# vpecanins/stm32f7-rtlsdr

Measured on AMD Instinct MI355X. Metric: IQ MSamples/s through FIR+FM-demod+resample, higher is better.
Workload: dtype f32 audio; K2 = u8 x 24-bit fixed-point taps on the i8 matrix pipe, exact i32 sums, one f32 recombination (design Q); K3 / K4 f32; ill-conditioned phases recomputed with the f32 fmaf chain

## Files before the change

include/sdrfm_dev.h:

```cpp
#ifndef SDRFM_DEV_H
#define SDRFM_DEV_H

#include "sdrfm.h"

#ifdef __cplusplus
extern "C" {
#endif

float sdrfm_host_atan2f(float y, float x);
float sdrfm_host_discriminate(float yr, float yi, float pr, float pi);

int sdrfm_debug_discriminate(int device, const float* yr, const float* yi, const float* pr, const float* pi,
                             float* out_scalar, float* out_pair, uint32_t n);

int sdrfm_q_build(const float* h, uint32_t T, uint32_t D, int8_t* A, float* q, float* cst, uint32_t* first_chunk);

int sdrfm_q_guard(const float* h, uint32_t T, const float* g, uint32_t Ta, float* guard_r, float* guard_a);
int sdrfm_q_guard2(const float* h, uint32_t T, const float* g, uint32_t Ta, int worst_case, float* guard_r, float* guard_a);

int sdrfm_debug_q_guard(sdrfm_t* h, float* guard_r, float* guard_a, unsigned long long* lanes, unsigned long long* passes);

int sdrfm_debug_route(sdrfm_t* h, const uint8_t* mask, uint32_t* n_noisy, uint8_t* noisy_out);

int sdrfm_sink_chain_tables(float alpha, float* pc, float* w, float* dinv);

int sdrfm_debug_read_ceiling(int device, const void* const* bufs, uint32_t nbufs, size_t bytes_each, uint32_t passes, double* gbytes_per_s);

int sdrfm_debug_phase_cycles(sdrfm_t* h, unsigned long long* out8);
int sdrfm_debug_raw(sdrfm_t* h, unsigned long long* out560);
int sdrfm_dev_read_debug(sdrfm_t* h, unsigned long long* out, uint32_t n);
// ... 6 lines not shown
```

stm32f7-rtlsdr_amd/csrc/qtaps.c:

```c
#include <math.h>
#include <stdint.h>
#include <string.h>

#include "sdrfm_q_host.h"

int sdrfm_q_build(const float* h, uint32_t T, uint32_t D, int8_t* A, float* q_out, float* cst_out, uint32_t* first_chunk) {
  if (!h || !A || !q_out || !cst_out || !first_chunk) return -1;
  if (D < 2 || (D & 1u) || D > SDRFM_Q_MAX_D || T < 1 || T > 9 * D) return -1;
  double hmax = 0.0, hsum = 0.0;
  for (uint32_t k = 0; k < T; ++k) {
    if (!isfinite(h[k])) return -1;
    if (fabs((double)h[k]) > hmax) hmax = fabs((double)h[k]);
    hsum += (double)h[k];
  }
  if (hmax == 0.0) return -1;
  const double q = hmax / (double)SDRFM_Q_HMAX;
  const float qf = (float)q;
  if (!(qf > 0.0f) || !isfinite(65536.0f * qf)) return -1;
  int8_t dig[SDRFM_Q_DIGITS][9 * SDRFM_Q_MAX_D];
  for (uint32_t k = 0; k < T; ++k) {
    long long H = llround((double)h[k] / (double)qf);
    if (H > SDRFM_Q_HMAX) H = SDRFM_Q_HMAX;
    if (H < -SDRFM_Q_HMAX) H = -SDRFM_Q_HMAX;
    for (int t = 0; t < SDRFM_Q_DIGITS; ++t) {
// ... 13 lines not shown
        const uint32_t h2 = sl >> 3, q4 = (sl >> 1) & 3u, j = sl & 1u;
        const uint32_t kb = 128 * c + 32 * (l >> 4) + 16 * h2 + 4 * q4 + comp + 2 * j;
        const int k = (int)(8 * D + D * o + D - 1) - (int)(kb >> 1);
        if (kb >= 32 * D || k < 0 || k >= (int)T) continue;
        for (int t = 0; t < SDRFM_Q_DIGITS; ++t) {
          A[(((size_t)c * SDRFM_Q_DIGITS + t) * 64 + l) * 16 + sl] = dig[t][k];
          if (dig[t][k] != 0 && c < c0) c0 = c;
        }
      }
  *q_out = qf;
  *cst_out = (float)(0.5 * hsum);
  *first_chunk = c0;
  return 0;
}

int sdrfm_q_guard2(const float* h, uint32_t T, const float* g, uint32_t Ta, int worst_case, float* guard_r, float* guard_a) {
  if (!h || !g || !guard_r || !guard_a || T < 1 || Ta < 1) return -1;
  double habs = 0.0, hmax = 0.0, gmax = 0.0;
  for (uint32_t k = 0; k < T; ++k) { habs += fabs((double)h[k]); if (fabs((double)h[k]) > hmax) hmax = fabs((double)h[k]); }
  for (uint32_t k = 0; k < Ta; ++k) if (fabs((double)g[k]) > gmax) gmax = fabs((double)g[k]);
  if (!isfinite(habs) || !isfinite(gmax)) return -1;
  if (gmax == 0.0) { *guard_r = 0.0f; *guard_a = 4.0f; return 0; }
  const double P = 127.5 * habs, u = ldexp(1.0, -24);
  const double E = worst_case ? ((double)T + 4.0) * P * u + 64.0 * (double)T * (hmax / (double)SDRFM_Q_HMAX)
                              : 1.25 * sqrt((double)T) * P * u;
  *guard_r = (float)(2.0 * gmax * E / 5e-6);
  *guard_a = (float)(3.14159265358979323846 - 2.0 * 5e-6 / gmax);
  return 0;
}

// ... 4 lines not shown
```

stm32f7-rtlsdr_amd/csrc/sdrfm.hip:

```cpp
#include <hip/hip_runtime.h>
#include <hip/hip_ext.h>

#include <cmath>
#include <cstdint>
#include <cstdio>
#include <cstdlib>
#include <cstring>
#include <new>
#include <type_traits>

#include "../../include/sdrfm.h"
#include "../../include/sdrfm_dev.h"
#include "sdrfm_math.h"
#include "sdrfm_q.h"
#include "sdrfm_fm_call.h"
#include "sdrfm_fm_route.h"
#include "sdrfm_fm_plan.h"

#include "sdrfm_b.h"

static_assert(SDRFM_FM_Q_STEP_OUT == SDRFM_Q_STEP_OUT, "sdrfm_fm_call.h counts design Q's steps");
static_assert(SDRFM_FM_CHAIN_FIX == SDRFM_CHAIN_FIX, "sdrfm_fm_call.h sizes the runs of a launch with the sink's chain");

namespace {
// ... 750 lines not shown
  const FastVariant* fast_mix;
  char fast_s_name[64];
  uint32_t AB;
  unsigned long long* d_dbg;
  uint32_t warm_ahead;
  uint32_t dbg_launches;
  int fast_mode;
  uint32_t prio_balance;
  uint32_t end_prio;
  uint32_t stream_profile;
  char kernel_name[112];
  char generic_name[64];
  char fast_name[64];
  int8_t* d_qA;
  float q_scale, q_cst;
  uint32_t q_c0, q_nslot;
  char fast_q_name[64];
  float q_guard_r, q_guard_a;
  float* d_hpad;
  uint8_t* d_hist_q[2];
  unsigned int* d_qstat;
  bool yprev_exact, hist_q_valid;
  bool prev_by_q;
  FmRoute route;
  uint32_t* rt_pass_dev[SDRFM_Q_ADAPT_SETS]; uint32_t* rt_pass_host[SDRFM_Q_ADAPT_SETS]; uint32_t* rt_pass_host_dev[SDRFM_Q_ADAPT_SETS];
  hipStream_t rt_mon;
  hipEvent_t rt_rb_done[SDRFM_Q_ADAPT_SETS];
  hipEvent_t rt_win_evt[SDRFM_Q_ADAPT_SETS][3];
  uint32_t* rt_list_dev[2]; uint32_t* rt_list_host[2];
  hipEvent_t rt_applied[2];
// ... 282 lines not shown
  CR(hipMemcpy(h->d_g, gc, sizeof(float) * Ta, hipMemcpyHostToDevice));
#undef CR

  FmKnobs knobs = fm_read_knobs();
  FmPlanIn in;
  memset(&in, 0, sizeof(in));
  in.T = cfg->fir_taps; in.D = cfg->fir_decim; in.Ta = cfg->audio_taps; in.Da = cfg->audio_decim; in.n_streams = cfg->n_streams;
  in.force_generic = (cfg->flags & SDRFM_CFG_FORCE_GENERIC) != 0; in.bit_exact = (cfg->flags & SDRFM_CFG_BIT_EXACT) != 0;
  in.n_cu = (uint32_t)prop.multiProcessorCount;
  in.q_default_nslot = sdrfm_q_default_nslot(in.D);
  in.q_default_lds = sdrfm_q_lds_bytes(in.q_default_nslot, in.D, in.Da);
  if (!in.force_generic) in.taps = fm_tap_verdict(hc, in.T, gc, in.Ta, (cfg->flags & SDRFM_CFG_GUARD_WORST_CASE) != 0);
  const size_t q_tab_bytes = (size_t)SDRFM_Q_SPARSE_CHUNKS(in.D) * SDRFM_Q_DIGITS * 64 * 16;
  int8_t* q_tab = nullptr;
  float q_scale = 0.f, q_cst = 0.f;
  if (fm_plan_offers_q(in, knobs)) {
    q_tab = (int8_t*)malloc(q_tab_bytes);
    in.q_built = q_tab && sdrfm_q_build(hc, in.T, in.D, q_tab, &q_scale, &q_cst, &in.q_c0) == 0;
    const uint32_t nslot = fm_plan_q_nslot(in, knobs);
    in.q_lds = sdrfm_q_lds_bytes(nslot, in.D, in.Da);
    in.q_symbol = sdrfm_q_kernel_symbol(in.q_c0, nslot, in.D, in.Da);
    in.mix_lds = sdrfm_q_mix_lds(in.q_c0, nslot, in.D, in.Da, in.T, SDRFM_FM_MIX_R);
    if (in.mix_lds) in.mix_blocks_per_cu = sdrfm_q_mix_blocks_per_cu(in.q_c0, nslot, in.D, in.Da, in.T, SDRFM_FM_MIX_R);
  }
  FmRefused refused = {false, 0u};
  FmPlan plan;
  for (;;) {
    plan = fm_plan(in, knobs, refused);
    if (!plan.supported) break;
    if (plan.geo.has_q && !h->d_qA && !q_create(h, q_tab, q_tab_bytes)) {
      fprintf(stderr, "[sdrfm] the matrix-pipe kernel's tables or routing state could not be allocated: this handle runs the bit-exact kernels only\n");
      (void)hipGetLastError();
      q_free(h);
// ... 14 lines not shown
  free(q_tab);
  if (!plan.supported || (plan.lds_bytes > 64 * 1024 && hipFuncSetAttribute(reinterpret_cast<const void*>(k_generic), hipFuncAttributeMaxDynamicSharedMemorySize,
                                                                             (int)plan.lds_bytes) != hipSuccess)) { free_handle(h); return SDRFM_NOT_SUPPORTED; }
  h->geo = plan.geo;
  h->lds_bytes = plan.lds_bytes;
  h->fast = plan.fast >= 0 ? &kFastVariants[plan.fast] : nullptr;
  h->fast_s = plan.fast_s >= 0 ? &kFastVariants[plan.fast_s] : nullptr;
  h->fast_mix = plan.fast_mix >= 0 ? &kFastVariants[plan.fast_mix] : nullptr;
  if (h->geo.has_fast != (h->fast != nullptr) || h->geo.has_s != (h->fast_s != nullptr) || h->geo.has_mix_tile != (h->fast_mix != nullptr)) {
    fprintf(stderr, "[sdrfm] the plan's tiles and its geometry disagree\n");
    free_handle(h);
    return SDRFM_FAIL;
  }
  h->AB = plan.AB; h->warm_ahead = plan.warm_ahead; h->fast_mode = plan.fast_mode; h->stream_profile = plan.stream_profile ? 1u : 0u;
  h->prio_balance = knobs.prio_balance; h->end_prio = knobs.end_prio;
  if (plan.geo.has_q) { h->q_scale = q_scale; h->q_cst = q_cst; }
  h->q_c0 = plan.q_c0; h->q_nslot = plan.q_nslot; h->q_guard_r = plan.q_guard_r; h->q_guard_a = plan.q_guard_a;
  h->rt_off = knobs.q_no_adapt;
  snprintf(h->generic_name, sizeof(h->generic_name), "%s", plan.generic_name);
  snprintf(h->fast_name, sizeof(h->fast_name), "%s", plan.fast_name);
  snprintf(h->fast_s_name, sizeof(h->fast_s_name), "%s", plan.fast_s_name);
  snprintf(h->fast_q_name, sizeof(h->fast_q_name), "%s", plan.fast_q_name);
  snprintf(h->kernel_name, sizeof(h->kernel_name), "%s", plan.kernel_name);
  const int rc = sdrfm_reset(h);
  if (rc != SDRFM_OK) { free_handle(h); return rc; }
  *out = h;
  return SDRFM_OK;
}

void sdrfm_destroy(sdrfm_t* h) {
  if (!h) return;
// ... 303 lines not shown
  if (q_ok) {
    const uint32_t q_steps = fm_q_steps(M);
    SdrfmQParams q;
    q.iq_prev = nullptr; q.iq_prev_stride = 0; q.N_prev = 0;
    if (ovl) { q.iq_prev = h->prev_iq; q.iq_prev_stride = h->prev_stride; q.N_prev = h->prev_nbytes / 2; }
    q.iq = d_iq; q.iq_stride = iq_stride; q.audio = d_audio; q.audio_stride = audio_stride;
    q.yprev_in = p.yprev_in; q.yprev_out = p.yprev_out; q.hist_d_in = p.hist_d_in; q.hist_d_out = p.hist_d_out;
    q.hist_b_in = p.hist_b_in; q.hist_b_out = p.hist_b_out; q.hist_x_out = p.hist_x_out;
    q.A = h->d_qA; q.g = h->d_g; q.q0 = h->q_scale; q.q2 = 65536.0f * h->q_scale; q.cst = h->q_cst;
    q.T = c.fir_taps; q.N = N; q.M = M; q.A_out = A; q.steps_total = q_steps; q.n_streams = n_clean; q.dbg = nullptr; q.prio_by_age = ovl ? 0u : 1u;
    q.slist = list_dev;
    if (!h->hist_q_valid && !ovl && c.fir_taps > 1)
      HIP_TRY(hipMemcpy2DAsync(h->d_hist_q[h->cur] + 2 * (SDRFM_Q_TP - (c.fir_taps - 1)), 2 * SDRFM_Q_TP, p.hist_b_in, 2 * (size_t)(c.fir_taps - 1),
                               2 * (size_t)(c.fir_taps - 1), c.n_streams, hipMemcpyDeviceToDevice, h->stream), SDRFM_FAIL);
    q.hpad = h->d_hpad; q.hist_q_in = h->d_hist_q[h->cur]; q.hist_q_out = h->d_hist_q[h->cur ^ 1];
    q.guard_r = h->q_guard_r; q.guard_a = h->q_guard_a; q.yprev_exact = h->yprev_exact ? 1u : 0u; q.n_repaired = h->d_qstat;
    const FmRuns r = fm_q_runs(cl, split.q_total, n_clean, with_chain, h->runstate_cap, fm_chain_run_quads(g.Da));
    q.runs = r.runs;
    const bool carry = ovl && h->ovl_join_style;
    const FmRouteStop stop = fm_route_stop(rt, counting, k, carry);
    q.stream_pass = counting ? h->rt_pass_dev[stop.set] : nullptr;
    const hipEvent_t done = stop.evt == FM_ROUTE_OVL_DONE ? h->ovl_done[k] : stop.evt == FM_ROUTE_WINDOW_EVENT ? h->rt_win_evt[stop.set][k] : nullptr;
    with_chain = r.with_chain;
    if (with_chain) {
      chain.pcm = h->pcm_out; chain.pcm_stride = h->pcm_out_stride;
      if (h->pcm_no_audio) q.audio = nullptr;
      chain.run_call = h->chain_calls++;
      chain.runstate = h->d_runstate + (size_t)(chain.run_call % SDRFM_CHAIN_SETS) * h->runstate_cap;
    }
    if (fuse && with_chain) {
      HIP_TRY(sdrfm_q_launch_mix_pcm(q, chain, h->q_c0, h->q_nslot, c.fir_decim, c.audio_decim, pb, pb_blocks, g.mix_R, qs, nullptr), SDRFM_FAIL);
// ... 377 lines not shown
```

stm32f7-rtlsdr_amd/csrc/sdrfm_q.h:

```cpp
#ifndef SDRFM_Q_H
#define SDRFM_Q_H

#include <hip/hip_runtime.h>
#include <stdint.h>

#include "sdrfm_q_host.h"
#include "sdrfm_sink_chain.h"

struct SdrfmQParams {
  const uint8_t* iq;
  size_t iq_stride;
  const uint8_t* iq_prev;
  size_t iq_prev_stride;
  uint32_t N_prev;
  float* audio;
  size_t audio_stride;
  const float2* yprev_in;
  float2* yprev_out;
  const float* hist_d_in;
  float* hist_d_out;
  const uint8_t* hist_b_in;
  uint8_t* hist_b_out;
  float2* hist_x_out;
  const int8_t* A;
  const float* g;
  float q0, q2, cst;
  uint32_t T;
  uint32_t N, M, A_out;
  uint32_t steps_total;
  uint32_t runs;
  uint32_t n_streams;
  uint32_t prio_by_age;
  const float* hpad;
  const uint8_t* hist_q_in;
  uint8_t* hist_q_out;
  float guard_r;
  float guard_a;
  uint32_t yprev_exact;
  unsigned int* n_repaired;
  unsigned int* stream_pass;
  const uint32_t* slist;
  unsigned long long* dbg;
};

#define SDRFM_Q_D 10u
#define SDRFM_Q_DA 5u
#define SDRFM_Q_STEP_OUT 128u

bool sdrfm_q_geometry_ok(uint32_t d, uint32_t da);
uint32_t sdrfm_q_default_nslot(uint32_t d);
uint32_t sdrfm_q_lds_bytes(uint32_t nslot, uint32_t d, uint32_t da);
int sdrfm_q_blocks_per_cu(uint32_t first_chunk, uint32_t nslot, uint32_t d, uint32_t da);
hipError_t sdrfm_q_launch(const SdrfmQParams& p, uint32_t first_chunk, uint32_t nslot, uint32_t d, uint32_t da, hipStream_t stream, hipEvent_t done = nullptr);
bool sdrfm_q_has_pcm_chain(uint32_t first_chunk, uint32_t nslot, uint32_t d, uint32_t da);
hipError_t sdrfm_q_launch_pcm(const SdrfmQParams& p, const SdrfmSinkChain& t, uint32_t first_chunk, uint32_t nslot, uint32_t d, uint32_t da, hipStream_t stream,
                              hipEvent_t done = nullptr);
const char* sdrfm_q_kernel_symbol(uint32_t first_chunk, uint32_t nslot, uint32_t d, uint32_t da);
struct CallParams;
uint32_t sdrfm_q_mix_lds(uint32_t first_chunk, uint32_t nslot, uint32_t d, uint32_t da, uint32_t T, uint32_t b_R);
int sdrfm_q_mix_blocks_per_cu(uint32_t first_chunk, uint32_t nslot, uint32_t d, uint32_t da, uint32_t T, uint32_t b_R);
hipError_t sdrfm_q_launch_mix(const SdrfmQParams& q, uint32_t first_chunk, uint32_t nslot, uint32_t d, uint32_t da, const CallParams& b, uint32_t b_blocks,
                              uint32_t b_R, hipStream_t stream, hipEvent_t done);
hipError_t sdrfm_q_launch_mix_pcm(const SdrfmQParams& q, const SdrfmSinkChain& t, uint32_t first_chunk, uint32_t nslot, uint32_t d, uint32_t da, const CallParams& b,
                                  uint32_t b_blocks, uint32_t b_R, hipStream_t stream, hipEvent_t done);
hipError_t sdrfm_q_fix_yprev(const uint8_t* hist_q, const float* hpad, float2* yprev, uint32_t n_streams, const uint32_t* list, hipStream_t stream);

#endif
```

stm32f7-rtlsdr_amd/csrc/sdrfm_q.hip:

```cpp
#include <hip/hip_runtime.h>
#include <hip/hip_ext.h>

#include <cstddef>
#include <cstdint>
#include <type_traits>

#include "sdrfm_math.h"
#include "sdrfm_q.h"
#include "sdrfm_b.h"

typedef int qi4_t __attribute__((ext_vector_type(4)));
typedef int qi8_t __attribute__((ext_vector_type(8)));
typedef float qf2_t __attribute__((ext_vector_type(2)));
__device__ void q_raw_buffer_load_lds(qi4_t rsrc, __attribute__((address_space(3))) void* lds, int size, int voffset, int soffset,
                                      int offset, int aux) __asm("llvm.amdgcn.raw.buffer.load.lds");

namespace {

constexpr int QTA = (int)SDRFM_Q_TA;
constexpr int DB0 = 128;
constexpr int ABS = 4;
constexpr int ABW = 128 * ABS;
constexpr int FLW = 64 + 2;
#ifndef SDRFM_Q_GTAB
// ... 20 lines not shown
#ifndef SDRFM_Q_HO_RING
#define SDRFM_Q_HO_RING 1
#endif
#ifndef SDRFM_Q_K3
#define SDRFM_Q_K3 1
#endif
#ifndef SDRFM_Q_XORSKIP
#define SDRFM_Q_XORSKIP 1
#endif
#ifndef SDRFM_Q_PEEL
#define SDRFM_Q_PEEL 1
#endif
#ifndef SDRFM_Q_MICRO
#define SDRFM_Q_MICRO 1
#endif
#ifndef SDRFM_Q_AUX
#define SDRFM_Q_AUX 2
#endif
#ifndef SDRFM_Q_WQB
#define SDRFM_Q_WQB 4
#endif
constexpr int WQB = SDRFM_Q_WQB;
static_assert(WQB >= 4 && WQB <= 16 && 8 * WQB >= (int)SDRFM_Q_TA, "a warm-up holds the d history of a run's first audio output");

__device__ __forceinline__ float q_discriminate(float yr, float yi, float pr, float pi) {
  const float re = __builtin_fmaf(yr, pr, yi * pi);
  const float im = yi * pr - yr * pi;
  const float ax = __builtin_fabsf(re), ay = __builtin_fabsf(im);
  const float mx = __builtin_fmaxf(__builtin_fmaxf(ax, ay), 0x1p-120f), mn = __builtin_fminf(ax, ay);
  const float v = mn * __builtin_amdgcn_rcpf(mx);
  const float s2 = v * v;
  float q = 0x1.e34882p-8f;
  q = __builtin_fmaf(q, s2, -0x1.22fc74p-5f);
  q = __builtin_fmaf(q, s2, 0x1.509024p-4f);
  q = __builtin_fmaf(q, s2, -0x1.12688cp-3f);
  q = __builtin_fmaf(q, s2, 0x1.96c562p-3f);
  q = __builtin_fmaf(q, s2, -0x1.554086p-2f);
  float a = __builtin_fmaf(v, s2 * q, v);
  if (ay > ax) a = 0x1.921fb6p+0f - a;
  if (re < 0.0f) a = 0x1.921fb6p+1f - a;
  return __builtin_copysignf(a, im);
}

__device__ __forceinline__ float q_angle(float yr, float yi, float& mx_out) {
  const float ax = __builtin_fabsf(yr), ay = __builtin_fabsf(yi);
  const float mx = __builtin_fmaxf(__builtin_fmaxf(ax, ay), 0x1p-120f), mn = __builtin_fminf(ax, ay);
  mx_out = mx;
  const float v = mn * __builtin_amdgcn_rcpf(mx);
  const float s2 = v * v;
  float q = 0x1.e34882p-8f;
  q = __builtin_fmaf(q, s2, -0x1.22fc74p-5f);
  q = __builtin_fmaf(q, s2, 0x1.509024p-4f);
  q = __builtin_fmaf(q, s2, -0x1.12688cp-3f);
  q = __builtin_fmaf(q, s2, 0x1.96c562p-3f);
  q = __builtin_fmaf(q, s2, -0x1.554086p-2f);
  float a = __builtin_fmaf(v, s2 * q, v);
  if (ay > ax) a = 0x1.921fb6p+0f - a;
  if (yr < 0.0f) a = 0x1.921fb6p+1f - a;
  return __builtin_copysignf(a, yi);
}
__device__ __forceinline__ float q_wrap(float x) {
  float t = __builtin_fmaf(x, 0x1.45f306p-3f, 0x1.8p+23f);
  asm volatile("" : "+v"(t));
  const float k = t - 0x1.8p+23f;
  return __builtin_fmaf(k, -0x1.921fb6p+2f, x);
}

__device__ __forceinline__ unsigned q_pcm_word(float v) {
  const float c = __builtin_amdgcn_fmed3f(v, -32768.0f, 32767.0f);
  float t = c + 0x1.8p+23f;
  asm volatile("" : "+v"(t));
  return __builtin_amdgcn_perm(__builtin_bit_cast(unsigned, t), __builtin_bit_cast(unsigned, t), 0x05040504u);
}

template <int N>
__device__ __forceinline__ void wait_vmcnt() {
  static_assert(N >= 0 && N < 16, "vmcnt immediate");
  __builtin_amdgcn_s_waitcnt(0x0f70 | N);
}

// ... 144 lines not shown
    constexpr int HSW = ALIGNED ? 0x70 : 0;
#ifdef SDRFM_Q_LDSXOR
    hb0 ^= 0x8080; hb1 ^= 0x8080;
#endif
    if (lane < HT) *reinterpret_cast<unsigned short*>(smem + ((PRE - 2 * HT + 2 * lane) ^ HSW)) = hb0;
    if (lane + 64 < HT) *reinterpret_cast<unsigned short*>(smem + ((PRE - 2 * HT + 2 * (lane + 64)) ^ HSW)) = hb1;
    if (lane < QTA - 1) db[DB0 + sigma - (QTA - 1) + lane] = hd0;
  }
#if SDRFM_Q_K3
  float cth = 0.0f;
  unsigned long long cfl = 0ull;
  if (!warm) {
    float mxp;
    const float tp = q_angle(cr, ci, mxp);
    cth = __builtin_bit_cast(float, __builtin_amdgcn_readfirstlane(__builtin_bit_cast(int, tp)));
    cfl = __builtin_amdgcn_ballot_w64(mxp < p.guard_r) & 1ull;
  }
#endif
  db[lane] = hz0;
  if (lane < 2 * QD) db[64 + lane] = hz1;
#if SDRFM_Q_GTAB
  if (lane < QTA) gt[lane] = gt0;
#endif
  __builtin_amdgcn_wave_barrier();
  int slot = 0;
  int ringoff = 0;
  int osm = 0;
  int mbase = o0;
  const int baddr = BLKB * n + 16 * g;
  int rdoff[ALIGNED ? 2 * NSC : 1];
  if constexpr (ALIGNED) {
// ... 31 lines not shown
    t_wait += __builtin_readcyclecounter() - tw0;
    if (t_first == 0) t_first = __builtin_amdgcn_s_memrealtime();
#endif
    if constexpr (ALIGNED) {
      const int ro0 = n == 0 ? 0 : ringoff;
#pragma unroll
      for (int c = 2 * C0; c < 2 * NSC; ++c) dst[c - 2 * C0] = *reinterpret_cast<const qi4_t*>(smem + rdoff[c] + (64 * c < BLKB ? ro0 : ringoff));
      if (lane < BLKB / 16) {
        const qi4_t hcp = *reinterpret_cast<const qi4_t*>(smem + PRE + ringoff + STEPB - BLKB + 16 * lane);
        *reinterpret_cast<qi4_t*>(smem + 16 * lane) = hcp;
      }
      __builtin_amdgcn_wave_barrier();
    } else {
      const unsigned char* wb = smem + baddr + ringoff;
#pragma unroll
      for (int c = 2 * C0; c < 2 * NSC; ++c) dst[c - 2 * C0] = *reinterpret_cast<const qi4_t*>(wb + 64 * c);
      if (ringoff + STEPB == RINGB) {
        if (lane < BLKB / 16) {
          const qi4_t hcp = *reinterpret_cast<const qi4_t*>(smem + PRE + RINGB - BLKB + 16 * lane);
          *reinterpret_cast<qi4_t*>(smem + 16 * lane) = hcp;
        }
        __builtin_amdgcn_wave_barrier();
      }
    }
    if constexpr (RINGB == 2 * STEPB) ringoff ^= STEPB;
    else ringoff = (ringoff + STEPB == RINGB) ? 0 : ringoff + STEPB;
  };
  auto refill_step = [&](int k) {
    asm volatile("s_waitcnt lgkmcnt(0)" ::: "memory");
    if constexpr (ALIGNED) {
#pragma unroll
// ... 216 lines not shown
        float* dst = db + DB0 + sigma + 128 * slot + 8 * (l & 15) + 2 * (l >> 4);
        dst[0] = sdrfm_discriminate(a[1].x, a[1].y, a[0].x, a[0].y);
        dst[1] = sdrfm_discriminate(a[2].x, a[2].y, a[1].x, a[1].y);
      }
    }
    R_PHASE(7, 0, 1);
    if (ln == 0) {
      cnt[0] += nrep;
      cnt[1] += 1u;
    }
    nflag = 0;
    R_PHASE(7, 32, 1);
  };
#ifdef SDRFM_Q_GUARD_L1
  float guard_r = 2.0f * p.guard_r, guard_a = p.guard_a;
#else
  float guard_r = p.guard_r, guard_a = p.guard_a;
#endif
  asm volatile("" : "+v"(guard_r), "+v"(guard_a));
#ifdef SDRFM_Q_SCALE_VGPR
  float q0v = p.q0, q2v = p.q2, cstv = p.cst;
  asm volatile("" : "+v"(q0v), "+v"(q2v), "+v"(cstv));
#else
  const float q0v = p.q0, q2v = p.q2, cstv = p.cst;
#endif
#if SDRFM_Q_MICRO && SDRFM_Q_K3
  int doff = (PRE + RINGB) + 4 * (DB0 + sigma + dlane);
  asm volatile("" : "+v"(doff));
#endif
  const int wrank = (int)(__builtin_amdgcn_s_getreg((3 << 11) | 4) & 15u);
  const int prio_at = p.prio_by_age ? nsteps / 2 : -1;
#if SDRFM_Q_PEEL
  auto step = [&](auto LAST_, const int kk) {
    constexpr bool LAST = decltype(LAST_)::value;
#else
  for (int kk = 0; kk < nsteps; ++kk) {
    const bool LAST = kk == nsteps - 1;
#endif
    if (kk == prio_at) {
// ... 18 lines not shown
        if (lane < 2 * QTP / 16)
          *reinterpret_cast<qi4_t*>(pp->hist_q_out + (size_t)(2 * QTP) * stream + 16 * lane) =
              *reinterpret_cast<const qi4_t*>(smem + PRE + ((Ge - 2 * QTP + 16 * lane) % RINGB));
      }
    }
#endif
    Q_PHASE(1);
    if (!(SDRFM_Q_PEEL && LAST)) refill_step(kk);
#ifdef SDRFM_Q_EARLYSTORE
    if (LAST && npend > 0) flush_audio();
#endif
    Q_PHASE(2);
    qi4_t acc[SDRFM_Q_DIGITS];
#pragma unroll
    for (int t = 0; t < SDRFM_Q_DIGITS; ++t) acc[t] = qi4_t{0, 0, 0, 0};
    [[maybe_unused]] constexpr int XM = (int)0x80808080;
#ifndef SDRFM_Q_LDSXOR
#pragma unroll
    for (int c = 0; c < NB - 1 + (NCH & 1 ? 0 : 1); ++c)
      B[c] = B[c] ^ ((SDRFM_Q_XORSKIP && QD == 10 && C0 == 0 && c == 0) ? qi4_t{0, XM, XM, XM} : qi4_t{XM, XM, XM, XM});
#endif
#pragma unroll
    for (int c = C0; c < NSC; ++c) {
      const qi4_t lo = B[2 * c - 2 * C0], hi = B[2 * c + 1 - 2 * C0];
      const qi8_t b = {lo.x, lo.y, lo.z, lo.w, hi.x, hi.y, hi.z, hi.w};
#pragma unroll
      for (int t = 0; t < SDRFM_Q_DIGITS; ++t) {
#if defined(SDRFM_Q_ABLATE) && (SDRFM_Q_ABLATE & 2)
        acc[t] += At[c - C0][t] & lo;
#else
        acc[t] = __builtin_amdgcn_smfmac_i32_16x16x128_i8(At[c - C0][t], b, acc[t], sidx, 0, 0);
#endif
      }
    }
    float y[4];
#pragma unroll
    for (int r = 0; r < 4; ++r) {
      const int s01 = acc[0][r] + acc[1][r] * 256;
      y[r] = __builtin_fmaf((float)s01, q0v, __builtin_fmaf((float)acc[2][r], q2v, cstv));
    }
#ifdef SDRFM_Q_PHASES
    asm volatile("" : "+v"(y[0]), "+v"(y[1]), "+v"(y[2]), "+v"(y[3]));
#endif
    Q_PHASE(3);
#if SDRFM_Q_K3
    float mx0, mx1;
    const float th1 = q_angle(y[2], y[3], mx1);
    float thp = __builtin_bit_cast(float, __builtin_amdgcn_ds_bpermute(srcaddr, __builtin_bit_cast(int, th1)));
    const float th0 = q_angle(y[0], y[1], mx0);
#if SDRFM_Q_MICRO
    asm("v_writelane_b32 %0, %1, 0" : "+v"(thp) : "s"(cth));
#else
    if (lane == 0) thp = cth;
#endif
#ifdef SDRFM_Q_PHASES
    asm volatile("" : "+v"(thp));
#endif
    Q_PHASE(4);
    cth = __builtin_bit_cast(float, __builtin_amdgcn_readlane(__builtin_bit_cast(int, th1), 63));
    const float d1 = q_wrap(th1 - th0);
    const float d0 = q_wrap(th0 - thp);
#else
    float pr = __builtin_bit_cast(float, __builtin_amdgcn_ds_bpermute(srcaddr, __builtin_bit_cast(int, y[2])));
    float pi = __builtin_bit_cast(float, __builtin_amdgcn_ds_bpermute(srcaddr, __builtin_bit_cast(int, y[3])));
    if (lane == 0) { pr = cr; pi = ci; }
#ifdef SDRFM_Q_PHASES
    asm volatile("" : "+v"(pr), "+v"(pi));
#endif
    Q_PHASE(4);
    cr = __builtin_bit_cast(float, __builtin_amdgcn_readlane(__builtin_bit_cast(int, y[2]), 63));
    ci = __builtin_bit_cast(float, __builtin_amdgcn_readlane(__builtin_bit_cast(int, y[3]), 63));
#if defined(SDRFM_Q_ABLATE) && (SDRFM_Q_ABLATE & 1)
    const float d0 = y[0] + pr + y[1] * pi, d1 = y[2] + y[3] * y[1] + y[0];
#else
    const float d1 = q_discriminate(y[2], y[3], y[0], y[1]);
    const float d0 = q_discriminate(y[0], y[1], pr, pi);
// ... 197 lines not shown
  }
#ifdef SDRFM_Q_STAMPS
  if (tsp && lane == 0) {
    tsp[0] = t_entry; tsp[1] = t_first; tsp[2] = t_loop; tsp[3] = __builtin_amdgcn_s_memrealtime(); tsp[4] = t_wait;
#ifdef SDRFM_Q_PHASES
    for (int i = 0; i < 8; ++i) tsp[8 + i] = t_ph[i];
#endif
    tsp[5] = (__builtin_amdgcn_s_getreg((3 << 11) | 20) & 7) | ((unsigned long long)__builtin_amdgcn_s_getreg((31 << 11) | 4) << 8);
    tsp[6] = (unsigned long long)nsteps; tsp[7] = __builtin_readcyclecounter() - c_entry;
  }
#endif
}


template <int C0, int NSLOT, int D, int DA>
__global__ void __launch_bounds__(64) __attribute__((amdgpu_waves_per_eu(D == 16 ? 3 : 4))) k_mfir(SdrfmQParams p) {
  mfir_body<C0, NSLOT, D, DA>(p, blockIdx.x);
}

template <int C0, int NSLOT, int D, int DA>
__global__ void __launch_bounds__(64) __attribute__((amdgpu_waves_per_eu(D == 16 ? 3 : 4))) k_mfir_pcm(QPcmArgs a) {
  mfir_body<C0, NSLOT, D, DA, true>(a.p, blockIdx.x);
}

template <int C0, int NSLOT, int D, int DA, int T, int R>
__global__ void __launch_bounds__(64) __attribute__((amdgpu_waves_per_eu(3, 4))) k_mix(SdrfmQParams q, CallParams b, uint32_t nb) {
  if (blockIdx.x < nb) fastb_body<T, D, R, (int)SDRFM_Q_TA, DA, 0>(b, blockIdx.x);
  else mfir_body<C0, NSLOT, D, DA>(q, blockIdx.x - nb);
}

struct MixPcmArgs { QPcmArgs qa; CallParams b; uint32_t nb; };
template <int C0, int NSLOT, int D, int DA, int T, int R>
__global__ void __launch_bounds__(64) __attribute__((amdgpu_waves_per_eu(3, 4))) k_mix_pcm(MixPcmArgs a) {
  if (blockIdx.x < a.nb) fastb_body<T, D, R, (int)SDRFM_Q_TA, DA, 0>(a.b, blockIdx.x);
  else mfir_body<C0, NSLOT, D, DA, true>(a.qa.p, blockIdx.x - a.nb);
}
// ... 107 lines not shown
}

uint32_t sdrfm_q_default_nslot(uint32_t d) { return d == 10 ? 5u : (d == 8 ? 4u : (d == 16 ? 8u : 0u)); }

bool sdrfm_q_geometry_ok(uint32_t d, uint32_t da) { return q_find(0, sdrfm_q_default_nslot(d), d, da) != nullptr; }

uint32_t sdrfm_q_lds_bytes(uint32_t nslot, uint32_t d, uint32_t da) {
  const QVariant* v = q_find(0, nslot, d, da);
  return v ? v->lds : 0u;
}

const char* sdrfm_q_kernel_symbol(uint32_t first_chunk, uint32_t nslot, uint32_t d, uint32_t da) {
  const QVariant* v = q_find(first_chunk, nslot, d, da);
  return v ? v->name : "";
}

int sdrfm_q_blocks_per_cu(uint32_t first_chunk, uint32_t nslot, uint32_t d, uint32_t da) {
  const QVariant* v = q_find(first_chunk, nslot, d, da);
  int nb = 0;
  if (!v || hipOccupancyMaxActiveBlocksPerMultiprocessor(&nb, reinterpret_cast<const void*>(v->k), 64, v->lds) != hipSuccess) return 0;
  return nb;
}

hipError_t sdrfm_q_fix_yprev(const uint8_t* hist_q, const float* hpad, float2* yprev, uint32_t n_streams, const uint32_t* list, hipStream_t stream) {
  hipLaunchKernelGGL(k_q_fix_yprev, dim3((n_streams + 63) / 64), dim3(64), 0, stream, hist_q, hpad, yprev, n_streams, list);
  return hipGetLastError();
}

hipError_t sdrfm_q_launch(const SdrfmQParams& p, uint32_t first_chunk, uint32_t nslot, uint32_t d, uint32_t da, hipStream_t stream, hipEvent_t done) {
  const QVariant* v = q_find(first_chunk, nslot, d, da);
// ... 57 lines not shown
```

stm32f7-rtlsdr_amd/csrc/sdrfm_q_host.h:

```cpp
#ifndef SDRFM_Q_HOST_H
#define SDRFM_Q_HOST_H

#include <stdint.h>

#ifdef __cplusplus
extern "C" {
#endif

#define SDRFM_Q_DIGITS 3
#define SDRFM_Q_HMAX (127 * 65793)
#define SDRFM_Q_MAX_D 16

#define SDRFM_Q_TA 32u
#define SDRFM_Q_TP 64u
#define SDRFM_Q_SPARSE_CHUNKS(D) (((D) + 3u) / 4u)

int sdrfm_q_build(const float* h, uint32_t T, uint32_t D, int8_t* A, float* q, float* cst, uint32_t* first_chunk);

int sdrfm_q_guard(const float* h, uint32_t T, const float* g, uint32_t Ta, float* guard_r, float* guard_a);
int sdrfm_q_guard2(const float* h, uint32_t T, const float* g, uint32_t Ta, int worst_case, float* guard_r, float* guard_a);

#ifdef __cplusplus
}
#endif
#endif
```

stm32f7-rtlsdr_amd/lib.py:

```python
import ctypes as C
import os

import numpy as np

_HERE = os.path.dirname(os.path.abspath(__file__))

STATUS = {
    0: "SDRFM_OK", 1: "SDRFM_BUSY", 2: "SDRFM_FAIL", 3: "SDRFM_NOT_SUPPORTED", 4: "SDRFM_UNRECOVERED_ERROR",
    16: "SDRFM_EINVAL", 17: "SDRFM_EODD", 18: "SDRFM_ECAPACITY", 19: "SDRFM_NO_DEVICE", 20: "SDRFM_ENOMEM",
}
OK, EINVAL, EODD, ECAPACITY, NO_DEVICE = 0, 16, 17, 18, 19
F_DEVICE_PTRS = 1
F_OVERLAP = 2
TUNE_SHARED_INPUT = 1

ABI_SYMBOLS = [
    "sdrfm_create", "sdrfm_destroy", "sdrfm_reset", "sdrfm_audio_count", "sdrfm_process", "sdrfm_process_batch",
    "sdrfm_set_stream", "sdrfm_synchronize", "sdrfm_flush", "sdrfm_flush_previous", "sdrfm_wait_previous", "sdrfm_process_batch_pcm", "sdrfm_kernel_name", "sdrfm_abi_version", "sdrfm_strerror",
    "sdrfm_wbfm_create", "sdrfm_wbfm_destroy", "sdrfm_wbfm_reset", "sdrfm_wbfm_audio_count", "sdrfm_wbfm_process_batch",
    "sdrfm_wbfm_set_stream", "sdrfm_wbfm_synchronize", "sdrfm_wbfm_kernel_name", "sdrfm_rtl_pack_fir", "sdrfm_rtl_resampler", "sdrfm_e4k_pll_params",
    "sdrfm_shard_range",
    "sdrfm_spectrum_create", "sdrfm_spectrum_destroy", "sdrfm_spectrum_process_batch", "sdrfm_spectrum_set_stream",
    "sdrfm_spectrum_synchronize", "sdrfm_spectrum_kernel_name",
    "sdrfm_pcm_deemph_s16", "sdrfm_pcm_alpha",
# ... 18 lines not shown
    "sdrfm_bcast_process_batch_metered_hist", "sdrfm_bcast_hist_kernel_name",
    "sdrfm_pcm_audio_meter_s16", "sdrfm_audio_meter_add", "sdrfm_audio_meter_report",
    "sdrfm_pcm_stereo_sink_meter_enable", "sdrfm_pcm_stereo_sink_meter_disable", "sdrfm_pcm_stereo_sink_meter_read",
    "sdrfm_loudness_default_coef", "sdrfm_loudness_check_coef", "sdrfm_loudness_check_domain", "sdrfm_pcm_loudness_s16", "sdrfm_loudness_gate_create", "sdrfm_loudness_gate_push",
    "sdrfm_loudness_gate_report", "sdrfm_loudness_gate_reset", "sdrfm_loudness_gate_free", "sdrfm_pcm_stereo_sink_loudness_enable",
    "sdrfm_pcm_stereo_sink_loudness_disable", "sdrfm_pcm_stereo_sink_loudness_read", "sdrfm_pcm_stereo_sink_loudness_get_state",
    "sdrfm_truepeak_default_coef", "sdrfm_truepeak_check_coef", "sdrfm_truepeak_limit", "sdrfm_pcm_truepeak_s16", "sdrfm_truepeak_add",
    "sdrfm_truepeak_report", "sdrfm_pcm_stereo_sink_truepeak_enable", "sdrfm_pcm_stereo_sink_truepeak_disable",
    "sdrfm_pcm_stereo_sink_truepeak_read",
    "sdrfm_pcm_rate_create", "sdrfm_pcm_rate_destroy", "sdrfm_pcm_rate_reset", "sdrfm_pcm_rate_set_step", "sdrfm_pcm_rate_count",
    "sdrfm_pcm_rate_process_batch", "sdrfm_pcm_rate_get_state", "sdrfm_pcm_rate_set_stream", "sdrfm_pcm_rate_synchronize",
    "sdrfm_pcm_rate_kernel_name", "sdrfm_pcm_rate_s16", "sdrfm_pcm_rate_check_coef",
]


TEST_HOOK_SYMBOLS = ["sdrfm_host_atan2f", "sdrfm_host_discriminate", "sdrfm_debug_discriminate", "sdrfm_q_build", "sdrfm_q_guard", "sdrfm_q_guard2", "sdrfm_debug_q_guard", "sdrfm_debug_read_ceiling", "sdrfm_debug_route", "sdrfm_sink_chain_tables"]
DEV_ONLY_SYMBOLS = ["sdrfm_debug_phase_cycles", "sdrfm_debug_raw", "sdrfm_dev_read_debug"]


class SdrfmError(RuntimeError):
    def __init__(self, status, where=""):
        self.status = int(status)
        name = STATUS.get(self.status, "status %d" % self.status)
        msg = ""
        try:
            msg = load_library().sdrfm_strerror(self.status).decode()
        except Exception:
            pass
        super().__init__("%s%s (%s)" % (where + ": " if where else "", name, msg))


# ... 196 lines not shown
    lib.sdrfm_strerror.argtypes = [C.c_int]
    lib.sdrfm_strerror.restype = C.c_char_p
    lib.sdrfm_host_atan2f.argtypes = [C.c_float, C.c_float]
    lib.sdrfm_host_atan2f.restype = C.c_float
    lib.sdrfm_host_discriminate.argtypes = [C.c_float] * 4
    lib.sdrfm_host_discriminate.restype = C.c_float
    lib.sdrfm_sink_chain_tables.argtypes = [C.c_float] + [C.POINTER(C.c_float)] * 3
    lib.sdrfm_sink_chain_tables.restype = C.c_int
    if dev:
        lib.sdrfm_debug_phase_cycles.argtypes = [vp, C.POINTER(C.c_uint64)]
        lib.sdrfm_debug_phase_cycles.restype = C.c_int
        lib.sdrfm_debug_raw.argtypes = [vp, C.POINTER(C.c_uint64)]
        lib.sdrfm_debug_raw.restype = C.c_int
    lib.sdrfm_q_build.argtypes = [vp, u32, u32, vp, C.POINTER(C.c_float), C.POINTER(C.c_float), u32p]
    lib.sdrfm_q_build.restype = C.c_int
    lib.sdrfm_debug_discriminate.argtypes = [C.c_int] + [vp] * 6 + [u32]
    lib.sdrfm_debug_discriminate.restype = C.c_int
    lib.sdrfm_q_guard.argtypes = [vp, u32, vp, u32, C.POINTER(C.c_float), C.POINTER(C.c_float)]
    lib.sdrfm_q_guard.restype = C.c_int
    lib.sdrfm_q_guard2.argtypes = [vp, u32, vp, u32, C.c_int, C.POINTER(C.c_float), C.POINTER(C.c_float)]
    lib.sdrfm_q_guard2.restype = C.c_int
    lib.sdrfm_debug_read_ceiling.argtypes = [C.c_int, C.POINTER(vp), u32, C.c_size_t, u32, C.POINTER(C.c_double)]
    lib.sdrfm_debug_read_ceiling.restype = C.c_int
    lib.sdrfm_debug_q_guard.argtypes = [vp, C.POINTER(C.c_float), C.POINTER(C.c_float), C.POINTER(C.c_uint64), C.POINTER(C.c_uint64)]
    lib.sdrfm_debug_q_guard.restype = C.c_int
    lib.sdrfm_debug_route.argtypes = [vp, C.POINTER(C.c_uint8), C.POINTER(C.c_uint32), C.POINTER(C.c_uint8)]
    lib.sdrfm_debug_route.restype = C.c_int
    lib.sdrfm_wbfm_create.argtypes = [C.POINTER(WbfmConfig), C.POINTER(vp)]
    lib.sdrfm_wbfm_create.restype = C.c_int
    lib.sdrfm_wbfm_destroy.argtypes = [vp]
# ... 274 lines not shown
```

Measured before the change: 2.558 million.

## Recombine Q-path FIR sums scale-free with integer seed and drop dead B-chunk load

Drops the per-output float scale and constant from the design-Q recombination. The 0.5*sum(h) constant becomes an integer seed, computed on the host and preloaded into the digit-0 accumulator. Because K3 works on differences of angles, the output is only combined as acc0 + 256*acc1 + 65536*acc2, and the guard radius is rescaled by the quantum to match. It also skips loading the last, all-zero B half-chunk when the chunk count is odd, and adds optional knobs for pinning constants to VGPRs and for occupancy, both off by default. The aim is fewer VALU ops and fewer LDS reads per step, at the cost of an int32 overflow check and a changed scale for the yprev history.

```diff
diff --git a/include/sdrfm_dev.h b/include/sdrfm_dev.h
--- a/include/sdrfm_dev.h
+++ b/include/sdrfm_dev.h
@@ -14,6 +14,8 @@
                              float* out_scalar, float* out_pair, uint32_t n);
 
 int sdrfm_q_build(const float* h, uint32_t T, uint32_t D, int8_t* A, float* q, float* cst, uint32_t* first_chunk);
+
+int sdrfm_q_seed(const float* h, uint32_t T, uint32_t D, int32_t* seed);
 
 int sdrfm_q_guard(const float* h, uint32_t T, const float* g, uint32_t Ta, float* guard_r, float* guard_a);
 int sdrfm_q_guard2(const float* h, uint32_t T, const float* g, uint32_t Ta, int worst_case, float* guard_r, float* guard_a);
diff --git a/stm32f7-rtlsdr_amd/csrc/qtaps.c b/stm32f7-rtlsdr_amd/csrc/qtaps.c
--- a/stm32f7-rtlsdr_amd/csrc/qtaps.c
+++ b/stm32f7-rtlsdr_amd/csrc/qtaps.c
@@ -1,5 +1,6 @@
 #include <math.h>
 #include <stdint.h>
+#include <stdlib.h>
 #include <string.h>
 
 #include "sdrfm_q_host.h"
@@ -51,6 +52,37 @@
   return 0;
 }
 
+int sdrfm_q_seed(const float* h, uint32_t T, uint32_t D, int32_t* seed_out) {
+  if (!h || !seed_out || D < 2 || (D & 1u) || D > SDRFM_Q_MAX_D || T < 1 || T > 9 * D) return -1;
+  double hmax = 0.0, hsum = 0.0;
+  for (uint32_t k = 0; k < T; ++k) {
+    if (!isfinite(h[k])) return -1;
+    if (fabs((double)h[k]) > hmax) hmax = fabs((double)h[k]);
+    hsum += (double)h[k];
+  }
+  if (hmax == 0.0) return -1;
+  const float qf = (float)(hmax / (double)SDRFM_Q_HMAX);
+  if (!(qf > 0.0f) || !isfinite(65536.0f * qf)) return -1;
+  long long sumH = 0, reach = 0;
+  for (uint32_t k = 0; k < T; ++k) {
+    long long H = llround((double)h[k] / (double)qf);
+    if (H > SDRFM_Q_HMAX) H = SDRFM_Q_HMAX;
+    if (H < -SDRFM_Q_HMAX) H = -SDRFM_Q_HMAX;
+    sumH += H;
+    const long long d0 = ((H + 128) % 256 + 256) % 256 - 128, H1 = (H - d0) / 256, d1 = ((H1 + 128) % 256 + 256) % 256 - 128;
+    reach += 128 * (llabs(d0) + 256 * llabs(d1));
+  }
+  long long seed = sumH / 2;
+  if (sumH & 1) {
+    const double want = 0.5 * hsum / (double)qf;
+    const long long lo = (sumH - 1) / 2;
+    seed = fabs((double)lo - want) <= fabs((double)(lo + 1) - want) ? lo : lo + 1;
+  }
+  if (llabs(seed) + reach > 2147483647LL) return -1;
+  *seed_out = (int32_t)seed;
+  return 0;
+}
+
 int sdrfm_q_guard2(const float* h, uint32_t T, const float* g, uint32_t Ta, int worst_case, float* guard_r, float* guard_a) {
   if (!h || !g || !guard_r || !guard_a || T < 1 || Ta < 1) return -1;
   double habs = 0.0, hmax = 0.0, gmax = 0.0;
diff --git a/stm32f7-rtlsdr_amd/csrc/sdrfm.hip b/stm32f7-rtlsdr_amd/csrc/sdrfm.hip
--- a/stm32f7-rtlsdr_amd/csrc/sdrfm.hip
+++ b/stm32f7-rtlsdr_amd/csrc/sdrfm.hip
@@ -788,6 +788,7 @@
   char fast_name[64];
   int8_t* d_qA;
   float q_scale, q_cst;
+  int32_t q_seed;
   uint32_t q_c0, q_nslot;
   char fast_q_name[64];
   float q_guard_r, q_guard_a;
@@ -1100,9 +1101,10 @@
   const size_t q_tab_bytes = (size_t)SDRFM_Q_SPARSE_CHUNKS(in.D) * SDRFM_Q_DIGITS * 64 * 16;
   int8_t* q_tab = nullptr;
   float q_scale = 0.f, q_cst = 0.f;
+  int32_t q_seed = 0;
   if (fm_plan_offers_q(in, knobs)) {
     q_tab = (int8_t*)malloc(q_tab_bytes);
-    in.q_built = q_tab && sdrfm_q_build(hc, in.T, in.D, q_tab, &q_scale, &q_cst, &in.q_c0) == 0;
+    in.q_built = q_tab && sdrfm_q_build(hc, in.T, in.D, q_tab, &q_scale, &q_cst, &in.q_c0) == 0 && sdrfm_q_seed(hc, in.T, in.D, &q_seed) == 0;
     const uint32_t nslot = fm_plan_q_nslot(in, knobs);
     in.q_lds = sdrfm_q_lds_bytes(nslot, in.D, in.Da);
     in.q_symbol = sdrfm_q_kernel_symbol(in.q_c0, nslot, in.D, in.Da);
@@ -1147,7 +1149,7 @@
   }
   h->AB = plan.AB; h->warm_ahead = plan.warm_ahead; h->fast_mode = plan.fast_mode; h->stream_profile = plan.stream_profile ? 1u : 0u;
   h->prio_balance = knobs.prio_balance; h->end_prio = knobs.end_prio;
-  if (plan.geo.has_q) { h->q_scale = q_scale; h->q_cst = q_cst; }
+  if (plan.geo.has_q) { h->q_scale = q_scale; h->q_cst = q_cst; h->q_seed = q_seed; }
   h->q_c0 = plan.q_c0; h->q_nslot = plan.q_nslot; h->q_guard_r = plan.q_guard_r; h->q_guard_a = plan.q_guard_a;
   h->rt_off = knobs.q_no_adapt;
   snprintf(h->generic_name, sizeof(h->generic_name), "%s", plan.generic_name);
@@ -1481,7 +1483,7 @@
       HIP_TRY(hipMemcpy2DAsync(h->d_hist_q[h->cur] + 2 * (SDRFM_Q_TP - (c.fir_taps - 1)), 2 * SDRFM_Q_TP, p.hist_b_in, 2 * (size_t)(c.fir_taps - 1),
                                2 * (size_t)(c.fir_taps - 1), c.n_streams, hipMemcpyDeviceToDevice, h->stream), SDRFM_FAIL);
     q.hpad = h->d_hpad; q.hist_q_in = h->d_hist_q[h->cur]; q.hist_q_out = h->d_hist_q[h->cur ^ 1];
-    q.guard_r = h->q_guard_r; q.guard_a = h->q_guard_a; q.yprev_exact = h->yprev_exact ? 1u : 0u; q.n_repaired = h->d_qstat;
+    q.guard_r = h->q_guard_r; q.guard_a = h->q_guard_a; q.seed = h->q_seed; q.guard_rq = h->q_guard_r / h->q_scale; q.yprev_exact = h->yprev_exact ? 1u : 0u; q.n_repaired = h->d_qstat;
     const FmRuns r = fm_q_runs(cl, split.q_total, n_clean, with_chain, h->runstate_cap, fm_chain_run_quads(g.Da));
     q.runs = r.runs;
     const bool carry = ovl && h->ovl_join_style;
diff --git a/stm32f7-rtlsdr_amd/csrc/sdrfm_q.h b/stm32f7-rtlsdr_amd/csrc/sdrfm_q.h
--- a/stm32f7-rtlsdr_amd/csrc/sdrfm_q.h
+++ b/stm32f7-rtlsdr_amd/csrc/sdrfm_q.h
@@ -36,6 +36,8 @@
   uint8_t* hist_q_out;
   float guard_r;
   float guard_a;
+  int32_t seed;
+  float guard_rq;
   uint32_t yprev_exact;
   unsigned int* n_repaired;
   unsigned int* stream_pass;
@@ -56,6 +58,7 @@
 hipError_t sdrfm_q_launch_pcm(const SdrfmQParams& p, const SdrfmSinkChain& t, uint32_t first_chunk, uint32_t nslot, uint32_t d, uint32_t da, hipStream_t stream,
                               hipEvent_t done = nullptr);
 const char* sdrfm_q_kernel_symbol(uint32_t first_chunk, uint32_t nslot, uint32_t d, uint32_t da);
+double sdrfm_q_yprev_scale(float q0);
 struct CallParams;
 uint32_t sdrfm_q_mix_lds(uint32_t first_chunk, uint32_t nslot, uint32_t d, uint32_t da, uint32_t T, uint32_t b_R);
 int sdrfm_q_mix_blocks_per_cu(uint32_t first_chunk, uint32_t nslot, uint32_t d, uint32_t da, uint32_t T, uint32_t b_R);
diff --git a/stm32f7-rtlsdr_amd/csrc/sdrfm_q.hip b/stm32f7-rtlsdr_amd/csrc/sdrfm_q.hip
--- a/stm32f7-rtlsdr_amd/csrc/sdrfm_q.hip
+++ b/stm32f7-rtlsdr_amd/csrc/sdrfm_q.hip
@@ -58,6 +58,19 @@
 #ifndef SDRFM_Q_MICRO
 #define SDRFM_Q_MICRO 1
 #endif
+#ifndef SDRFM_Q_SCALEFREE
+#define SDRFM_Q_SCALEFREE 1
+#endif
+#ifndef SDRFM_Q_NOB6
+#define SDRFM_Q_NOB6 1
+#endif
+#ifndef SDRFM_Q_CVGPR
+#define SDRFM_Q_CVGPR 0
+#endif
+#ifndef SDRFM_Q_W3
+#define SDRFM_Q_W3 0
+#endif
+static_assert(!SDRFM_Q_SCALEFREE || SDRFM_Q_K3, "the scale-free recombination rests on K3 as a difference of angles");
 #ifndef SDRFM_Q_AUX
 #define SDRFM_Q_AUX 2
 #endif
@@ -86,28 +99,35 @@
   return __builtin_copysignf(a, im);
 }
 
-__device__ __forceinline__ float q_angle(float yr, float yi, float& mx_out) {
+struct QK {
+  float c[6] = {0x1.e34882p-8f, -0x1.22fc74p-5f, 0x1.509024p-4f, -0x1.12688cp-3f, 0x1.96c562p-3f, -0x1.554086p-2f};
+  float w[3] = {0x1.45f306p-3f, 0x1.8p+23f, -0x1.921fb6p+2f};
+  float hpi = 0x1.921fb6p+0f, pi = 0x1.921fb6p+1f;
+  float k16 = 65536.0f;
+  int xm = (int)0x80808080;
+};
+__device__ __forceinline__ float q_angle(float yr, float yi, float& mx_out, const QK& K = QK{}) {
   const float ax = __builtin_fabsf(yr), ay = __builtin_fabsf(yi);
   const float mx = __builtin_fmaxf(__builtin_fmaxf(ax, ay), 0x1p-120f), mn = __builtin_fminf(ax, ay);
   mx_out = mx;
   const float v = mn * __builtin_amdgcn_rcpf(mx);
   const float s2 = v * v;
-  float q = 0x1.e34882p-8f;
-  q = __builtin_fmaf(q, s2, -0x1.22fc74p-5f);
-  q = __builtin_fmaf(q, s2, 0x1.509024p-4f);
-  q = __builtin_fmaf(q, s2, -0x1.12688cp-3f);
-  q = __builtin_fmaf(q, s2, 0x1.96c562p-3f);
-  q = __builtin_fmaf(q, s2, -0x1.554086p-2f);
+  float q = K.c[0];
+  q = __builtin_fmaf(q, s2, K.c[1]);
+  q = __builtin_fmaf(q, s2, K.c[2]);
+  q = __builtin_fmaf(q, s2, K.c[3]);
+  q = __builtin_fmaf(q, s2, K.c[4]);
+  q = __builtin_fmaf(q, s2, K.c[5]);
   float a = __builtin_fmaf(v, s2 * q, v);
-  if (ay > ax) a = 0x1.921fb6p+0f - a;
-  if (yr < 0.0f) a = 0x1.921fb6p+1f - a;
+  if (ay > ax) a = K.hpi - a;
+  if (yr < 0.0f) a = K.pi - a;
   return __builtin_copysignf(a, yi);
 }
-__device__ __forceinline__ float q_wrap(float x) {
-  float t = __builtin_fmaf(x, 0x1.45f306p-3f, 0x1.8p+23f);
+__device__ __forceinline__ float q_wrap(float x, const QK& K = QK{}) {
+  float t = __builtin_fmaf(x, K.w[0], K.w[1]);
   asm volatile("" : "+v"(t));
-  const float k = t - 0x1.8p+23f;
-  return __builtin_fmaf(k, -0x1.921fb6p+2f, x);
+  const float k = t - K.w[1];
+  return __builtin_fmaf(k, K.w[2], x);
 }
 
 __device__ __forceinline__ unsigned q_pcm_word(float v) {
@@ -282,7 +302,11 @@
     float mxp;
     const float tp = q_angle(cr, ci, mxp);
     cth = __builtin_bit_cast(float, __builtin_amdgcn_readfirstlane(__builtin_bit_cast(int, tp)));
+#if SDRFM_Q_SCALEFREE
+    cfl = __builtin_amdgcn_ballot_w64(mxp < (p.yprev_exact ? p.guard_r : p.guard_rq)) & 1ull;
+#else
     cfl = __builtin_amdgcn_ballot_w64(mxp < p.guard_r) & 1ull;
+#endif
   }
 #endif
   db[lane] = hz0;
@@ -344,7 +368,7 @@
     } else {
       const unsigned char* wb = smem + baddr + ringoff;
 #pragma unroll
-      for (int c = 2 * C0; c < 2 * NSC; ++c) dst[c - 2 * C0] = *reinterpret_cast<const qi4_t*>(wb + 64 * c);
+      for (int c = 2 * C0; c < 2 * NSC - ((SDRFM_Q_NOB6 && (NCH & 1)) ? 1 : 0); ++c) dst[c - 2 * C0] = *reinterpret_cast<const qi4_t*>(wb + 64 * c);
       if (ringoff + STEPB == RINGB) {
         if (lane < BLKB / 16) {
           const qi4_t hcp = *reinterpret_cast<const qi4_t*>(smem + PRE + RINGB - BLKB + 16 * lane);
@@ -591,15 +615,28 @@
   };
 #ifdef SDRFM_Q_GUARD_L1
   float guard_r = 2.0f * p.guard_r, guard_a = p.guard_a;
+#elif SDRFM_Q_SCALEFREE
+  float guard_r = p.guard_rq, guard_a = p.guard_a;
 #else
   float guard_r = p.guard_r, guard_a = p.guard_a;
 #endif
   asm volatile("" : "+v"(guard_r), "+v"(guard_a));
+  QK K;
+  if constexpr ((SDRFM_Q_CVGPR & 1) != 0) asm volatile("" : "+v"(K.k16));
+  if constexpr ((SDRFM_Q_CVGPR & 2) != 0) asm volatile("" : "+v"(K.c[0]), "+v"(K.c[1]), "+v"(K.c[2]), "+v"(K.c[3]), "+v"(K.c[4]), "+v"(K.c[5]));
+  if constexpr ((SDRFM_Q_CVGPR & 4) != 0) asm volatile("" : "+v"(K.w[0]), "+v"(K.w[1]), "+v"(K.w[2]));
+  if constexpr ((SDRFM_Q_CVGPR & 8) != 0) asm volatile("" : "+v"(K.hpi), "+v"(K.pi));
+  if constexpr ((SDRFM_Q_CVGPR & 16) != 0) asm volatile("" : "+v"(K.xm));
+#if SDRFM_Q_SCALEFREE
+  const int seed1 = __builtin_amdgcn_readfirstlane(p.seed);
+  unsigned long long seed2 = (unsigned long long)(unsigned)seed1 * 0x100000001ull;
+  asm volatile("" : "+v"(seed2));
+#endif
 #ifdef SDRFM_Q_SCALE_VGPR
   float q0v = p.q0, q2v = p.q2, cstv = p.cst;
   asm volatile("" : "+v"(q0v), "+v"(q2v), "+v"(cstv));
 #else
-  const float q0v = p.q0, q2v = p.q2, cstv = p.cst;
+  [[maybe_unused]] const float q0v = p.q0, q2v = p.q2, cstv = p.cst;
 #endif
 #if SDRFM_Q_MICRO && SDRFM_Q_K3
   int doff = (PRE + RINGB) + 4 * (DB0 + sigma + dlane);
@@ -648,7 +685,18 @@
     qi4_t acc[SDRFM_Q_DIGITS];
 #pragma unroll
     for (int t = 0; t < SDRFM_Q_DIGITS; ++t) acc[t] = qi4_t{0, 0, 0, 0};
-    [[maybe_unused]] constexpr int XM = (int)0x80808080;
+#if SDRFM_Q_SCALEFREE
+    {
+      typedef unsigned long long ql2_t __attribute__((ext_vector_type(2)));
+      unsigned long long a0, a1, z0, z1, z2, z3;
+      asm volatile("v_mov_b64 %0, %6\n\tv_mov_b64 %1, %6\n\tv_mov_b64 %2, 0\n\tv_mov_b64 %3, 0\n\tv_mov_b64 %4, 0\n\tv_mov_b64 %5, 0"
+                   : "=&v"(a0), "=&v"(a1), "=&v"(z0), "=&v"(z1), "=&v"(z2), "=&v"(z3) : "v"(seed2));
+      acc[0] = __builtin_bit_cast(qi4_t, ql2_t{a0, a1});
+      acc[1] = __builtin_bit_cast(qi4_t, ql2_t{z0, z1});
+      acc[2] = __builtin_bit_cast(qi4_t, ql2_t{z2, z3});
+    }
+#endif
+    [[maybe_unused]] const int XM = K.xm;
 #ifndef SDRFM_Q_LDSXOR
 #pragma unroll
     for (int c = 0; c < NB - 1 + (NCH & 1 ? 0 : 1); ++c)
@@ -656,7 +704,11 @@
 #endif
 #pragma unroll
     for (int c = C0; c < NSC; ++c) {
-      const qi4_t lo = B[2 * c - 2 * C0], hi = B[2 * c + 1 - 2 * C0];
+      const qi4_t lo = B[2 * c - 2 * C0];
+      qi4_t hi = B[2 * c + 1 - 2 * C0];
+      if constexpr (SDRFM_Q_NOB6 && (NCH & 1)) {
+        if (c == NSC - 1) asm volatile("" : "=v"(hi));
+      }
       const qi8_t b = {lo.x, lo.y, lo.z, lo.w, hi.x, hi.y, hi.z, hi.w};
 #pragma unroll
       for (int t = 0; t < SDRFM_Q_DIGITS; ++t) {
@@ -671,7 +723,11 @@
 #pragma unroll
     for (int r = 0; r < 4; ++r) {
       const int s01 = acc[0][r] + acc[1][r] * 256;
+#if SDRFM_Q_SCALEFREE
+      y[r] = __builtin_fmaf((float)acc[2][r], K.k16, (float)s01);
+#else
       y[r] = __builtin_fmaf((float)s01, q0v, __builtin_fmaf((float)acc[2][r], q2v, cstv));
+#endif
     }
 #ifdef SDRFM_Q_PHASES
     asm volatile("" : "+v"(y[0]), "+v"(y[1]), "+v"(y[2]), "+v"(y[3]));
@@ -679,9 +735,9 @@
     Q_PHASE(3);
 #if SDRFM_Q_K3
     float mx0, mx1;
-    const float th1 = q_angle(y[2], y[3], mx1);
+    const float th1 = q_angle(y[2], y[3], mx1, K);
     float thp = __builtin_bit_cast(float, __builtin_amdgcn_ds_bpermute(srcaddr, __builtin_bit_cast(int, th1)));
-    const float th0 = q_angle(y[0], y[1], mx0);
+    const float th0 = q_angle(y[0], y[1], mx0, K);
 #if SDRFM_Q_MICRO
     asm("v_writelane_b32 %0, %1, 0" : "+v"(thp) : "s"(cth));
 #else
@@ -692,8 +748,8 @@
 #endif
     Q_PHASE(4);
     cth = __builtin_bit_cast(float, __builtin_amdgcn_readlane(__builtin_bit_cast(int, th1), 63));
-    const float d1 = q_wrap(th1 - th0);
-    const float d0 = q_wrap(th0 - thp);
+    const float d1 = q_wrap(th1 - th0, K);
+    const float d0 = q_wrap(th0 - thp, K);
 #else
     float pr = __builtin_bit_cast(float, __builtin_amdgcn_ds_bpermute(srcaddr, __builtin_bit_cast(int, y[2])));
     float pi = __builtin_bit_cast(float, __builtin_amdgcn_ds_bpermute(srcaddr, __builtin_bit_cast(int, y[3])));
@@ -921,12 +977,12 @@
 
 
 template <int C0, int NSLOT, int D, int DA>
-__global__ void __launch_bounds__(64) __attribute__((amdgpu_waves_per_eu(D == 16 ? 3 : 4))) k_mfir(SdrfmQParams p) {
+__global__ void __launch_bounds__(64) __attribute__((amdgpu_waves_per_eu((D == 16 || (SDRFM_Q_W3 && D == 10)) ? 3 : 4))) k_mfir(SdrfmQParams p) {
   mfir_body<C0, NSLOT, D, DA>(p, blockIdx.x);
 }
 
 template <int C0, int NSLOT, int D, int DA>
-__global__ void __launch_bounds__(64) __attribute__((amdgpu_waves_per_eu(D == 16 ? 3 : 4))) k_mfir_pcm(QPcmArgs a) {
+__global__ void __launch_bounds__(64) __attribute__((amdgpu_waves_per_eu((D == 16 || (SDRFM_Q_W3 && D == 10)) ? 3 : 4))) k_mfir_pcm(QPcmArgs a) {
   mfir_body<C0, NSLOT, D, DA, true>(a.p, blockIdx.x);
 }
 
@@ -1064,6 +1120,8 @@
   const QVariant* v = q_find(first_chunk, nslot, d, da);
   return v ? v->name : "";
 }
+
+double sdrfm_q_yprev_scale(float q0) { return SDRFM_Q_SCALEFREE ? (double)q0 : 1.0; }
 
 int sdrfm_q_blocks_per_cu(uint32_t first_chunk, uint32_t nslot, uint32_t d, uint32_t da) {
   const QVariant* v = q_find(first_chunk, nslot, d, da);
diff --git a/stm32f7-rtlsdr_amd/csrc/sdrfm_q_host.h b/stm32f7-rtlsdr_amd/csrc/sdrfm_q_host.h
--- a/stm32f7-rtlsdr_amd/csrc/sdrfm_q_host.h
+++ b/stm32f7-rtlsdr_amd/csrc/sdrfm_q_host.h
@@ -17,6 +17,8 @@
 
 int sdrfm_q_build(const float* h, uint32_t T, uint32_t D, int8_t* A, float* q, float* cst, uint32_t* first_chunk);
 
+int sdrfm_q_seed(const float* h, uint32_t T, uint32_t D, int32_t* seed);
+
 int sdrfm_q_guard(const float* h, uint32_t T, const float* g, uint32_t Ta, float* guard_r, float* guard_a);
 int sdrfm_q_guard2(const float* h, uint32_t T, const float* g, uint32_t Ta, int worst_case, float* guard_r, float* guard_a);
 
diff --git a/stm32f7-rtlsdr_amd/lib.py b/stm32f7-rtlsdr_amd/lib.py
--- a/stm32f7-rtlsdr_amd/lib.py
+++ b/stm32f7-rtlsdr_amd/lib.py
@@ -56,7 +56,7 @@
 ]
 
 
-TEST_HOOK_SYMBOLS = ["sdrfm_host_atan2f", "sdrfm_host_discriminate", "sdrfm_debug_discriminate", "sdrfm_q_build", "sdrfm_q_guard", "sdrfm_q_guard2", "sdrfm_debug_q_guard", "sdrfm_debug_read_ceiling", "sdrfm_debug_route", "sdrfm_sink_chain_tables"]
+TEST_HOOK_SYMBOLS = ["sdrfm_host_atan2f", "sdrfm_host_discriminate", "sdrfm_debug_discriminate", "sdrfm_q_build", "sdrfm_q_seed", "sdrfm_q_guard", "sdrfm_q_guard2", "sdrfm_debug_q_guard", "sdrfm_debug_read_ceiling", "sdrfm_debug_route", "sdrfm_sink_chain_tables"]
 DEV_ONLY_SYMBOLS = ["sdrfm_debug_phase_cycles", "sdrfm_debug_raw", "sdrfm_dev_read_debug"]
 
 
@@ -283,6 +283,8 @@
         lib.sdrfm_debug_raw.restype = C.c_int
     lib.sdrfm_q_build.argtypes = [vp, u32, u32, vp, C.POINTER(C.c_float), C.POINTER(C.c_float), u32p]
     lib.sdrfm_q_build.restype = C.c_int
+    lib.sdrfm_q_seed.argtypes = [vp, u32, u32, C.POINTER(C.c_int32)]
+    lib.sdrfm_q_seed.restype = C.c_int
     lib.sdrfm_debug_discriminate.argtypes = [C.c_int] + [vp] * 6 + [u32]
     lib.sdrfm_debug_discriminate.restype = C.c_int
     lib.sdrfm_q_guard.argtypes = [vp, u32, vp, u32, C.POINTER(C.c_float), C.POINTER(C.c_float)]
```

Measured after the change: 2.589 million, median of 6. +1.2%, better.
